# kije/HSLU_I.BA_RAYTRACING.F2501_raytracer

Hardware: AMD Instinct MI355X
Metric: Mray/s (primary+secondary, rays counted as the reference casts them), semesterbild@high_resolution (higher is better)
Workload: dtype f32; 1 GPU; semesterbild@high_resolution+anti_aliasing+soft_shadows (text.obj); width=1620, height=1350, rays_per_frame=34992000, rays_traced_per_frame=19683000, pixels_written=1768966, objects=14578, lights=50, parallelism=tiles48x48/1gpu, frames_in_flight=2, build_id=a7677b40f149b919-p0s0w0o6, queue_bytes=0, scene_budget_bytes=2147483648, phases=0

## Files before the change

hslu_i/ba_raytracing/f2501_raytracer_amd/csrc/rt_api.cpp:

```cpp
#include <hip/hip_runtime.h>

#include <algorithm>
#include <chrono>
#include <cmath>
#include <cstdio>
#include <cstdlib>
#include <cstring>
#include <string>
#include <vector>

#include "rt_cell_resolve.h"
#include "rt_host.h"

static void trace_point(hipStream_t stream, const char* what, uint32_t a = 0, uint32_t b = 0, uint32_t c = 0);
#define RC_TRY(expr) do { const int rc_ = (expr); if (rc_ != RT_OK) return rc_; } while (0)

extern "C" {

#ifndef RT_BUILD_ID
#define RT_BUILD_ID "unknown"
#endif
const char* rt_build_id(void) { return RT_BUILD_ID; }

int rt_selftest_exact_math(int device, const float* in, float* out_sqrt, float* out_rcp, uint32_t n) {
// ... 16 lines not shown
  if (e1 != hipSuccess || e2 != hipSuccess) return fail(RT_ERR_HIP, "selftest copy failed");
  return RT_OK;
}

int rt_device_count(void) {
  int n = 0;
  if (hipGetDeviceCount(&n) != hipSuccess) return 0;
  return n;
}

void rt_scene_destroy(rt_scene* s) {
  if (!s) return;
  (void)hipSetDevice(s->device);
  if (s->tables_ev) (void)hipEventDestroy(s->tables_ev);
  for (hipEvent_t e : s->frame_ev)
    if (e) (void)hipEventDestroy(e);
  for (auto& w : s->ws) {
    if (w.cnt_ev) (void)hipEventDestroy(w.cnt_ev);
    if (w.cnt_host) (void)hipHostFree(w.cnt_host);
    if (w.fork_ev) (void)hipEventDestroy(w.fork_ev);
    w.acc.release();
    for (auto& l : w.lane) {
      if (l.stream) (void)hipStreamSynchronize(l.stream), (void)hipStreamDestroy(l.stream);
      if (l.done_ev) (void)hipEventDestroy(l.done_ev);
      for (int k = 0; k < 2; k++) {
        if (l.shade_stream[k]) (void)hipStreamSynchronize(l.shade_stream[k]), (void)hipStreamDestroy(l.shade_stream[k]);
        if (l.shade_done[k]) (void)hipEventDestroy(l.shade_done[k]);
      }
      for (hipEvent_t e : l.level_ev) (void)hipEventDestroy(e);
      if (l.hit_ev) (void)hipEventDestroy(l.hit_ev);
      for (DevBuf* b : {&l.queues, &l.qcount, &l.trace_ws, &l.hard, &l.hitrec, &l.sets}) b->release();
    }
  }
  for (DevBuf* b : {&s->blob, &s->aa, &s->cloud, &s->counters, &s->suplist, &s->fb, &s->aux_rgb, &s->costmap, &s->aux_id, &s->aux_t, &s->flag_geo, &s->flags, &s->cell_lists, &s->resolve_work, &s->progress_fb, &s->rays_argb})
    b->release();
  rt_scene_release_update(s);
  delete s;
}

static int upload(DevBuf& b, const void* src, size_t bytes) {
  int rc = b.ensure(bytes);
  if (rc != RT_OK) return rc;
  if (bytes) {
    hipError_t e = hipMemcpy(b.p, src, bytes, hipMemcpyHostToDevice);
    if (e != hipSuccess) return fail(RT_ERR_HIP, "hipMemcpy H2D failed: %s", hipGetErrorString(e));
  }
  return RT_OK;
}

int rt_scene_create(const rt_scene_desc* d, int device, rt_scene** out) {
  if (!d || !out) return fail(RT_ERR_INVALID_ARG, "null argument");
  *out = nullptr;
  int rc = rt_check_scene_desc(d);
  if (rc != RT_OK) return rc;
  if ((rc = rt_open_device(device)) != RT_OK) return rc;

  rt_scene* s = new rt_scene();
  s->device = device;
  s->budget = d->device_budget_bytes ? d->device_budget_bytes : RT_SCENE_BUDGET_DEFAULT;
  RtPackedScene pk;
  rc = rt_pack_scene(d, s->budget, &pk);
  if (rc == RT_OK && pk.n_cells) {
    rc = upload(s->flag_geo, pk.flag_geo.data(), pk.flag_geo.size() * 4);
    if (rc == RT_OK) rc = s->flags.ensure((size_t)pk.n_cells * 2 + 64);
  }
  if (rc == RT_OK) rc = s->counters.ensure(RT_SLOTS * RT_COUNTER_REPLICAS * 16 * sizeof(unsigned long long));
  if (rc == RT_OK) rc = upload(s->blob, pk.blob.data(), pk.blob.size());
// ... 2 lines not shown
  if (rc == RT_OK) {
    rt_sah_packed(pk, s->sah_created, nullptr);
    s->sah_tri_cost = d->bvh.tri_cost > 0.f ? d->bvh.tri_cost : 2.0f;
  }
  if (rc != RT_OK) {
    rt_scene_destroy(s);
    return rc;
  }
  s->dev = pk.dev;
  s->dev.base = (const char*)s->blob.p;
  s->info = pk.info;
  s->n_cells = pk.n_cells;
  s->n_tri_cells = pk.n_tri_cells;
  s->bytes_bvh = pk.bytes_bvh;
  s->max_leaf = pk.max_leaf;
  memcpy(s->aabb_lo, pk.aabb_lo, sizeof(s->aabb_lo));
  memcpy(s->aabb_hi, pk.aabb_hi, sizeof(s->aabb_hi));
  *out = s;
  return RT_OK;
}

int rt_scene_bvh_info(const rt_scene* s, rt_bvh_info* out) {
  if (!s || !out) return fail(RT_ERR_INVALID_ARG, "null argument");
  *out = s->info;
  return RT_OK;
}

int rt_scene_memory_info(const rt_scene* s, rt_scene_info* out) {
  if (!s || !out) return fail(RT_ERR_INVALID_ARG, "null argument");
  memset(out, 0, sizeof(*out));
  out->bytes_bvh = s->bytes_bvh;
  out->bytes_geometry = s->blob.cap > s->bytes_bvh ? s->blob.cap - s->bytes_bvh : 0;
  out->bytes_flags = s->flags.cap + s->flag_geo.cap;
  out->bytes_cell_lists = s->cell_lists.cap + s->resolve_work.cap;
  out->bytes_tables = s->aa.cap + s->cloud.cap + s->counters.cap + s->suplist.cap + s->costmap.cap;
  for (const auto& w : s->ws) {
    out->bytes_workspace += w.bytes();
    for (const auto& l : w.lane) out->bytes_workspace += l.qcount.cap;
  }
  out->bytes_frames = s->fb.cap + s->aux_rgb.cap + s->aux_id.cap + s->aux_t.cap + s->progress_fb.cap + s->rays_argb.cap;
  out->bytes_total = out->bytes_geometry + out->bytes_bvh + out->bytes_flags + out->bytes_cell_lists + out->bytes_tables + out->bytes_workspace +
                     out->bytes_frames;
  out->budget_bytes = s->budget;
  out->n_receiver_cells = s->n_cells;
  out->cell_lists_built = s->cell_lists_built ? 1u : 0u;
  return RT_OK;
}

}

int rt_validate_params(const rt_params* p) {
  if (!p) return fail(RT_ERR_INVALID_ARG, "null params");
  if (p->abi_version != RT_ABI_VERSION)
    return fail(RT_ERR_INVALID_ARG, "rt_params.abi_version %u != %u", p->abi_version, RT_ABI_VERSION);
  if (p->width == 0 || p->height == 0) return fail(RT_ERR_INVALID_ARG, "empty frame");
  if ((uint64_t)p->width * p->height > 0x7FFFFFFFull) return fail(RT_ERR_INVALID_ARG, "frame too large");
  if (p->win_w && (p->win_x0 + (uint64_t)p->win_w > p->width || p->win_y0 + (uint64_t)p->win_h > p->height || !p->win_h))
    return fail(RT_ERR_INVALID_ARG, "window outside the frame");
  if ((p->flags & RT_FLAG_ANTI_ALIASING) && p->aa_rays > 0 && !p->aa_offsets)
    return fail(RT_ERR_INVALID_ARG, "aa_offsets missing");
  if (p->light_mult > 1 && (!p->cloud_sets || p->n_cloud_sets == 0))
    return fail(RT_ERR_INVALID_ARG, "cloud_sets missing");
  if (p->n_ranks > 1 && p->rank >= p->n_ranks) return fail(RT_ERR_INVALID_ARG, "rank out of range");
  if (p->n_ranks > 1 && p->tile_size != 0 && p->tile_size < 16) return fail(RT_ERR_UNSUPPORTED, "tile_size < 16");
  if (p->traversal > RT_TRAVERSAL_LINEAR) return fail(RT_ERR_INVALID_ARG, "unknown traversal mode");
  if (p->max_depth_reflection > RT_MAX_DEPTH || p->max_depth_refraction > RT_MAX_DEPTH)
    return fail(RT_ERR_UNSUPPORTED, "recursion depth > %u", RT_MAX_DEPTH);
// ... 87 lines not shown
    if (new_table) s->cloud_host.assign(p->cloud_sets, p->cloud_sets + n);
    s->cloud_ball_f[0] = p->fw, s->cloud_ball_f[1] = p->fh, s->cloud_ball_f[2] = p->fd;
    rt_scale_cloud(s->cloud_host.data(), n, s->cloud_ball_f, &s->cloud_scaled, s->cloud_ball);
    HIP_TRY(hipMemcpyAsync(s->cloud.p, s->cloud_scaled.data(), n / 3 * 16, hipMemcpyHostToDevice, up.stream));
  }
  P->cloud_sets = (const float4*)s->cloud.p;
  memcpy(P->cloud_centre, s->cloud_ball, 12);
  P->cloud_delta = s->cloud_ball[3];
  rt_beam_constants(p->eps_distance, P);
  const uint32_t cap = p->tuning.shadow_candidate_cap;
  P->cand_cap = cap == RT_CAND_CAP_NONE ? 0u : (cap ? cap : 64u);
  return RT_OK;
}

static int prepare_receiver_flags(rt_scene* s, const rt_params* p, TableUpload& up, RtDevParams* P) {
  hipStream_t stream = up.stream;
  P->recv_flags = nullptr;
  if (p->tuning.no_receiver_flags || P->cand_cap == 0u) s->notes |= RT_NOTE_RECV_FLAGS_OFF_TUNING;
  if (!s->n_cells || !(P->cloud_delta > 0.0f)) s->notes |= RT_NOTE_RECV_FLAGS_OFF_SCENE;
  if (s->dev.n_lights > 8u) s->notes |= RT_NOTE_RECV_FLAGS_OFF_LIGHTS;
  if (p->traversal != RT_TRAVERSAL_BVH) s->notes |= RT_NOTE_RECV_FLAGS_OFF_TRAVERSAL;
  if (p->flags & RT_FLAG_BACKFACE_CULLING) s->notes |= RT_NOTE_RECV_FLAGS_OFF_CULLING;
  if (!p->tuning.no_receiver_flags && P->cand_cap != 0u && s->n_cells && s->dev.n_lights <= 8u && p->traversal == RT_TRAVERSAL_BVH &&
      !(p->flags & RT_FLAG_BACKFACE_CULLING) && P->cloud_delta > 0.0f) {
    const float key[8] = {P->beam_delta, p->eps_distance, P->cloud_centre[0], P->cloud_centre[1], P->cloud_centre[2], 1.f, 0.f, 0.f};
    if (memcmp(key, s->flags_key, sizeof(key)) != 0) {
      RC_TRY(up.begin());
      RtDevParams B = *P;
      B.flag_out = (uint16_t*)s->flags.p;
      B.flag_geo = (const float4*)s->flag_geo.p;
      B.n_cells = s->n_cells;
      B.n_tri_cells = s->n_tri_cells;
      s->cell_lists_built = false;
      B.cell_list_out = nullptr;
      const size_t list_bytes = (size_t)s->n_cells * s->dev.n_lights * 16u;
      size_t free_b = 0, total_b = 0;
      const size_t flag_bytes = s->flags.cap + s->flag_geo.cap;
      if (s->dev.n_slots <= 65533u && flag_bytes + list_bytes <= s->budget && hipMemGetInfo(&free_b, &total_b) == hipSuccess &&
          list_bytes <= (free_b + s->cell_lists.cap) / 4 && s->cell_lists.ensure(list_bytes + 64) == RT_OK) {
        HIP_TRY(hipMemsetAsync(s->cell_lists.p, 0xFF, list_bytes, stream));
        B.cell_list_out = (uint16_t*)s->cell_lists.p;
        s->cell_lists_built = true;
      }
      if (!s->cell_lists_built) s->cell_lists.release();
      hipError_t e = (hipError_t)rt_launch_flags(s->dev, B, stream);
      if (e != hipSuccess) return fail(RT_ERR_HIP, "rt_flags_kernel launch failed: %s", hipGetErrorString(e));
      trace_point(stream, "rt_flags_kernel: cells, lights, lists", s->n_cells, s->dev.n_lights, s->cell_lists_built ? 1u : 0u);
      static const char* const prune_env = getenv("RT_CELL_PRUNE");
      static const bool prune_off = prune_env && *prune_env == '0';
      if (s->cell_lists_built && !prune_off) {
        RtCellPruneArgs a{};
        a.flag_geo = (const float*)s->flag_geo.p;
        a.lists = (uint16_t*)s->cell_lists.p;
        a.flags = (uint16_t*)s->flags.p;
        a.n_cells = s->n_cells, a.n_tri_cells = s->n_tri_cells;
        memcpy(a.cloud_centre, P->cloud_centre, 12);
        a.beam_delta = P->beam_delta, a.beam_eps_o = P->beam_eps_o;
        a.mode = RT_PRUNE_FULL;
        e = (hipError_t)rt_launch_cell_prune(s->dev, a, stream);
        if (e != hipSuccess) return fail(RT_ERR_HIP, "rt_cell_prune_kernel launch failed: %s", hipGetErrorString(e));
        trace_point(stream, "rt_cell_prune_kernel: cells, lights", s->n_cells, s->dev.n_lights, 0u);
        static const char* const resolve_env = getenv("RT_CELL_RESOLVE");
        static const bool resolve_off = resolve_env && *resolve_env == '0';
        RtCellResolveArgs r{};
        const size_t temp_bytes = resolve_off ? 0 : rt_cell_resolve_temp_bytes(s->n_cells, s->budget - flag_bytes - list_bytes, &r.chunk_cells);
        if (temp_bytes && s->resolve_work.ensure(temp_bytes) == RT_OK) {
          r.cell = a;
          r.eps_push = P->beam_eps_push, r.eps_ulp = P->beam_eps_ulp;
          r.work = (uint32_t*)s->resolve_work.p;
          e = (hipError_t)rt_launch_cell_resolve(s->dev, r, stream);
          if (e != hipSuccess) return fail(RT_ERR_HIP, "rt_cell_resolve_kernel launch failed: %s", hipGetErrorString(e));
          trace_point(stream, "rt_cell_resolve_kernel: cells, lights, cells per chunk", s->n_cells, s->dev.n_lights, r.chunk_cells);
        } else {
          s->resolve_work.release();
        }
      }
      if (!s->cell_lists_built) s->resolve_work.release();
      memcpy(s->flags_key, key, sizeof(key));
    }
    P->recv_flags = (const uint16_t*)s->flags.p;
    if (s->cell_lists_built && !p->tuning.no_cell_lists) P->cell_lists = (const uint4*)s->cell_lists.p;
  }
  if (!P->cell_lists) s->notes |= RT_NOTE_CELL_LISTS_OFF;
  return RT_OK;
}

static void copy_frame_shape(rt_scene* s, const rt_params* p, uint32_t* argb_dev, const rt_aux* aux_dev, RtDevParams* P) {
  P->max_depth_reflection = p->max_depth_reflection;
  P->max_depth_refraction = p->max_depth_refraction;
  s->sort_bits_wanted = p->tuning.sort_bits;
  s->lanes_wanted = p->tuning.sub_frames;
  s->phases_wanted = p->tuning.phases;
  s->levels_wanted = p->tuning.levels;
  if (p->win_w) {
    P->win_x0 = p->win_x0, P->win_y0 = p->win_y0, P->win_w = p->win_w, P->win_h = p->win_h;
  } else {
    P->win_x0 = P->win_y0 = 0;
    P->win_w = p->width;
    P->win_h = p->height;
  }
  P->tile_size = p->tile_size ? p->tile_size : 48u;
  P->n_ranks = p->n_ranks;
  P->rank = p->rank;
  P->traversal = p->traversal;
  P->argb = argb_dev;
  if (aux_dev) {
    P->aux_rgb = aux_dev->rgb;
    P->aux_hit_id = aux_dev->hit_id;
    P->aux_hit_t = aux_dev->hit_t;
  }
}

static int take_frame_slot(rt_scene* s, const rt_params* p, hipStream_t stream, RtDevParams* P) {
  int blk = -1, oldest = 0, same = -1;
// ... 767 lines not shown
```

hslu_i/ba_raytracing/f2501_raytracer_amd/csrc/rt_cell_resolve.cpp:

```cpp
#include <hip/hip_runtime_api.h>

#include "rt_cell_resolve.h"
#include "rt_scene_pack.h"

void rt_cell_resolve_packed(const RtPackedScene& pk, RtCellResolveArgs a) {
  if (pk.dev.n_lights == 0u || pk.dev.n_lights > 8u || pk.flag_geo.empty()) return;
  a.cell.flag_geo = pk.flag_geo.data();
  a.cell.n_cells = a.cell.n_cells < pk.n_cells ? a.cell.n_cells : pk.n_cells;
  a.cell.n_tri_cells = pk.n_tri_cells;
  const char* base = (const char*)pk.blob.data();
  const uint32_t nl = pk.dev.n_lights;
  for (uint32_t c = 0; c < a.cell.n_cells; c++)
    rt_cell_resolve_cell(pk.dev, base, a, c, a.cell.lists + (size_t)c * nl * RT_PRUNE_LIST_SLOTS, a.cell.flags + c, a.counts ? a.counts + (size_t)c * nl : nullptr);
}

size_t rt_cell_resolve_temp_bytes(uint32_t n_cells, size_t budget_left, uint32_t* chunk_cells) {
  *chunk_cells = 0u;
  const size_t cap = budget_left < ((size_t)64u << 20) ? budget_left : ((size_t)64u << 20);
  if (n_cells == 0u || cap < 4096u + 4u * 256u) return 0;
  size_t chunk = (cap - 4096u) / 4u;
  if (chunk > n_cells) chunk = n_cells;
  if (((size_t)n_cells + chunk - 1u) / chunk > 1024u) return 0;
  *chunk_cells = (uint32_t)chunk;
  return 4096u + 4u * chunk;
}
```

hslu_i/ba_raytracing/f2501_raytracer_amd/csrc/rt_cell_resolve.h:

```cpp
#pragma once

#include "rt_cell_prune.h"

#define RT_RESOLVE_NEAR_CENTRE 0x100u
#define RT_RESOLVE_NO_INFLATE 0x200u
#define RT_RESOLVE_NO_NEAR 0x400u

struct RtCellResolveArgs {
  RtCellPruneArgs cell;
  float eps_push, eps_ulp;
  uint32_t* work;
  uint32_t chunk_cells;
  uint8_t* counts;
};

struct RtResolveCell {
  float pm[3], pt[8][3];
  float rho, scale;
};

RT_HD static inline bool rt_resolve_cell_setup(const RtDevScene& sc, const char* base, const RtCellPruneArgs& a, uint32_t c, RtResolveCell& K) {
  float extra;
  if (!rt_prune_cell_hull(sc, base, a, c, K.pm, K.pt, &extra)) return false;
  float r = 0.0f, scale = rt_fadd(rt_prune_norm1(K.pm), extra);
  for (int k = 0; k < 8; k++) {
    float dk[3];
    rt_prune_sub(K.pt[k], K.pm, dk);
    r = fmaxf(r, rt_prune_norm(dk));
    scale = fmaxf(scale, rt_fadd(rt_prune_norm1(K.pt[k]), extra));
  }
  K.rho = rt_fadd(rt_fadd(rt_fmul(r, 1.0001f), rt_fmul(2e-6f, scale)), a.beam_eps_o);
  K.scale = scale;
  return true;
}
RT_HD static inline void rt_resolve_beam(const RtDevScene& sc, const char* base, const RtCellPruneArgs& a, const RtResolveCell& K, uint32_t l, RtPruneBeam& B) {
  const float* lights = (const float*)(base + sc.off_lights);
  B.p[0] = K.pm[0], B.p[1] = K.pm[1], B.p[2] = K.pm[2];
  B.rho = K.rho;
  for (int x = 0; x < 3; x++) B.c[x] = rt_fadd(lights[8u * l + x], a.cloud_centre[x]);
  rt_prune_sub(B.c, B.p, B.dseg);
  B.delta = rt_fadd(a.beam_delta, rt_fmul(2e-6f, rt_fadd(K.scale, rt_prune_norm1(B.c))));
  B.lenp = rt_fadd(rt_fadd(rt_prune_norm(B.dseg), B.delta), B.rho);
}

RT_HD static inline bool rt_resolve_near_rule(const RtPruneBeam& B, const RtResolveCell& K, const RtCellResolveArgs& a, const float* q) {
  const float v1[3] = {q[0], q[1], q[2]}, X[3] = {q[9], q[10], q[11]};
  float b[3];
// ... 66 lines not shown
      if (next <= node) return false;
      node = next;
    }
    if (k >= n) return true;
    const uint32_t slot = first + k;
    k++;
    if (slot >= sc.n_slots || slot >= RT_PRUNE_LIST_OVERFLOW) return false;
    const float* q = isect + 12u * (size_t)slot;
    if (rt_prune_rule(B, q, mode & 0xFFu)) continue;
    if (!(mode & RT_RESOLVE_NO_NEAR) && rt_resolve_near_rule(B, K, a, q)) continue;
    if (!keep(slot)) return true;
  }
}

RT_HD static inline bool rt_cell_resolve_wanted(const uint16_t* list, uint32_t n_lights) {
  bool any = false;
  for (uint32_t l = 0; l < n_lights && l < 8u; l++) any = any || list[(size_t)l * RT_PRUNE_LIST_SLOTS] == RT_PRUNE_LIST_OVERFLOW;
  return any;
}

RT_HD static inline void rt_cell_resolve_cell(const RtDevScene& sc, const char* base, const RtCellResolveArgs& a, uint32_t c, uint16_t* list, uint16_t* flag,
                                              uint8_t* counts) {
  if (!rt_cell_resolve_wanted(list, sc.n_lights)) return;
  RtResolveCell K;
  if (!rt_resolve_cell_setup(sc, base, a.cell, c, K)) return;
  uint32_t fl = *flag;
  bool fl_changed = false;
  for (uint32_t l = 0; l < sc.n_lights && l < 8u; l++) {
    uint16_t* w = list + (size_t)l * RT_PRUNE_LIST_SLOTS;
    if (w[0] != RT_PRUNE_LIST_OVERFLOW) continue;
    RtPruneBeam B;
    rt_resolve_beam(sc, base, a.cell, K, l, B);
    uint32_t n = 0;
    uint16_t out[RT_PRUNE_LIST_SLOTS];
    const bool count_all = counts != nullptr;
    const bool ok = rt_resolve_walk(sc, base, a, K, B, [&](uint32_t slot) {
      if (n < RT_PRUNE_LIST_SLOTS) out[n] = (uint16_t)slot;
      n++;
      return n <= RT_PRUNE_LIST_SLOTS || count_all;
    });
    if (!ok) continue;
    if (counts) counts[l] = (uint8_t)(n < 255u ? n : 255u);
    if (n > RT_PRUNE_LIST_SLOTS) continue;
    for (uint32_t k = n; k < RT_PRUNE_LIST_SLOTS; k++) out[k] = (uint16_t)RT_PRUNE_LIST_END;
    memcpy(__builtin_assume_aligned(w, 16), out, 16);
    if (n == 0u) fl |= 1u << l, fl_changed = true;
  }
  if (fl_changed) *flag = (uint16_t)fl;
}

struct RtPackedScene;
void rt_cell_resolve_packed(const RtPackedScene& pk, RtCellResolveArgs a);
size_t rt_cell_resolve_temp_bytes(uint32_t n_cells, size_t budget_left, uint32_t* chunk_cells);
int rt_launch_cell_resolve(const RtDevScene& sc, const RtCellResolveArgs& a, void* stream);
```

hslu_i/ba_raytracing/f2501_raytracer_amd/csrc/rt_cell_resolve.hip:

```cpp
#include <hip/hip_runtime.h>

#include "rt_cell_resolve.h"

#define RT_CELL_RESOLVE_WG 256u
#define RT_CELL_RESOLVE_COUNTERS 1024u

__global__ __launch_bounds__(RT_CELL_RESOLVE_WG) void rt_cell_resolve_find_kernel(const uint16_t* lists, uint32_t n_lights, uint32_t cell0, uint32_t cell1,
                                                                                  uint32_t* counter, uint32_t* work) {
  const uint32_t c = cell0 + blockIdx.x * RT_CELL_RESOLVE_WG + threadIdx.x;
  const bool has = c < cell1 && rt_cell_resolve_wanted(lists + (size_t)c * n_lights * RT_PRUNE_LIST_SLOTS, n_lights);
  const unsigned long long m = __ballot(has);
  if (!m) return;
  const uint32_t lane = threadIdx.x & 63u, leader = (uint32_t)__ffsll((long long)m) - 1u;
  uint32_t at = 0u;
  if (lane == leader) at = atomicAdd(counter, (uint32_t)__popcll(m));
  at = (uint32_t)__shfl((int)at, (int)leader);
  if (has) work[at + (uint32_t)__popcll(m & ((1ull << lane) - 1ull))] = c;
}

__global__ __launch_bounds__(RT_CELL_RESOLVE_WG) void rt_cell_resolve_kernel(RtDevScene sc, RtCellResolveArgs a, const uint32_t* counter, const uint32_t* work) {
  const uint32_t i = blockIdx.x * RT_CELL_RESOLVE_WG + threadIdx.x;
  if (i >= *counter || i >= a.chunk_cells) return;
  const uint32_t c = work[i];
  if (c >= a.cell.n_cells) return;
  rt_cell_resolve_cell(sc, sc.base, a, c, a.cell.lists + (size_t)c * sc.n_lights * RT_PRUNE_LIST_SLOTS, a.cell.flags + c,
                       a.counts ? a.counts + (size_t)c * sc.n_lights : nullptr);
}

int rt_launch_cell_resolve(const RtDevScene& sc, const RtCellResolveArgs& a, void* stream) {
  const uint32_t n = a.cell.n_cells, chunk = a.chunk_cells;
  if (n == 0u || sc.n_lights == 0u || sc.n_lights > 8u || sc.n_thr == 0u) return 0;
  if (!a.work || chunk == 0u || ((size_t)n + chunk - 1u) / chunk > RT_CELL_RESOLVE_COUNTERS) return (int)hipErrorInvalidValue;
  hipStream_t st = (hipStream_t)stream;
  hipError_t e = hipMemsetAsync(a.work, 0, RT_CELL_RESOLVE_COUNTERS * 4u, st);
  if (e != hipSuccess) return (int)e;
  uint32_t* list = a.work + RT_CELL_RESOLVE_COUNTERS;
  uint32_t k = 0;
  for (uint32_t c0 = 0; c0 < n; k++) {
    const uint32_t c1 = n - c0 > chunk ? c0 + chunk : n;
    const dim3 grid((c1 - c0 + RT_CELL_RESOLVE_WG - 1u) / RT_CELL_RESOLVE_WG);
    hipLaunchKernelGGL(rt_cell_resolve_find_kernel, grid, dim3(RT_CELL_RESOLVE_WG), 0, st, a.cell.lists, sc.n_lights, c0, c1, a.work + k, list);
    hipLaunchKernelGGL(rt_cell_resolve_kernel, grid, dim3(RT_CELL_RESOLVE_WG), 0, st, sc, a, a.work + k, list);
    if ((e = hipGetLastError()) != hipSuccess) return (int)e;
    c0 = c1;
  }
  return 0;
}
```

hslu_i/ba_raytracing/f2501_raytracer_amd/csrc/rt_host.h:

```cpp
#pragma once

#include <hip/hip_runtime.h>

#include <string>
#include <vector>

#include "rt_closest.h"
#include "rt_multihit.h"
#include "rt_ray_key.h"
#include "rt_scene_pack.h"

#define fail rt_fail

#define HIP_TRY(expr)                                                                          \
  do {                                                                                         \
    hipError_t e_ = (expr);                                                                    \
    if (e_ != hipSuccess)                                                                      \
      return fail(e_ == hipErrorOutOfMemory ? RT_ERR_OOM : RT_ERR_HIP, "%s failed: %s", #expr, \
                  hipGetErrorString(e_));                                                      \
  } while (0)

#define RT_SLOTS 4
#define RT_LANES 2
#define RT_MAX_DEPTH 64u
// ... 219 lines not shown
    }
  } ws[RT_SLOTS];
  std::vector<uint32_t> sup_host;
  uint32_t sup_key[8] = {0, 0, 0, 0, 0, 0, 0, 0};
  DevBuf costmap;
  std::vector<uint32_t> cost_host;
  uint32_t cost_key[13] = {0, 0, 0, 0, 0, 0, 0, 0, 0, 0, 0, 0, 0};
  bool cost_valid = false, cost_wanted = false;
  uint32_t q_cap = 0, hard_cap = 0, batch_items = 0;
  StreamKey stream_key{};
  uint32_t key_gen = 0;
  uint32_t sticky_notes = 0;
  bool stream_verified = false;
  uint32_t est[RT_LANES][RT_CNT_STRIDE] = {{0}};
  bool est_valid = false;
  uint32_t sort_bits_wanted = 0;
  uint32_t lanes_wanted = 0;
  uint32_t phases_wanted = 0;
  uint32_t levels_wanted = 0;
  uint32_t calm_frames = 1u << 30;
  uint32_t tables_version = 0;
  float aabb_lo[3] = {0.f, 0.f, 0.f}, aabb_hi[3] = {1.f, 1.f, 1.f};
  std::vector<float> aa_host, cloud_host, cloud_scaled;
  std::vector<uint32_t> aa_table;
  uint32_t aa_unique = 0;
  bool aa_dedup = true;
  hipEvent_t tables_ev = nullptr;
  hipStream_t tables_stream = nullptr, last_stream = nullptr;
  bool tables_pending = false, rendered = false;
  float cloud_ball[4] = {0.f, 0.f, 0.f, -1.f};
  DevBuf flag_geo, flags;
  DevBuf cell_lists;
  DevBuf resolve_work;
  bool cell_lists_built = false;
  uint32_t n_cells = 0, n_tri_cells = 0;
  float flags_key[8] = {-1.f, 0.f, 0.f, 0.f, 0.f, 0.f, 0.f, 0.f};
  float cloud_ball_f[3] = {0.f, 0.f, 0.f};
  hipEvent_t frame_ev[RT_SLOTS] = {};
  bool frame_pending[RT_SLOTS] = {};
  uint32_t frame_seq[RT_SLOTS] = {};
  hipStream_t frame_stream[RT_SLOTS] = {};
  uint32_t frame_no = 0;
  int cur_block = 0, last_block = 0;
  int cur_ws = 0;
  int ws_last_block[RT_SLOTS] = {0, 1, 2, 3};
  uint32_t notes = 0;
  size_t queue_bytes = 0;
  RtRefitPlan plan;
  DevBuf plan_dev, upd_dev;
  size_t plan_off[5] = {0, 0, 0, 0, 0};
  void* upd_stage = nullptr;
  size_t upd_stage_cap = 0;
  float* upd_back = nullptr;
  uint64_t sah_created[2] = {0, 0};
  float sah_tri_cost = 2.0f;
  DevBuf sah_dev;
  uint32_t max_leaf = 4;
};


int rt_scene_upload_plan(rt_scene* s, const RtPackedScene& pk);
void rt_scene_release_update(rt_scene* s);

int rt_scene_wait_frames(rt_scene* s);

struct RtRebuildIn {
// ... 30 lines not shown
```

hslu_i/ba_raytracing/f2501_raytracer_amd/csrc/rt_internal.h:

```cpp
#pragma once

#include <stdint.h>

#include <vector>

#include "../../../../include/rt_hip.h"


struct RtNode {
  float lo0[3];
  uint32_t c0;
  float hi0[3];
  uint32_t n0;
  float lo1[3];
  uint32_t c1;
  float hi1[3];
  uint32_t n1;
};
static_assert(sizeof(RtNode) == 64, "node must be 64 bytes");

struct RtThrNode {
  float lo[3];
  uint32_t skip;
  float hi[3];
// ... 26 lines not shown
  uint32_t off_tri_shade;
  uint32_t off_tri_id;
  uint32_t off_materials;
  uint32_t off_lights;
  uint32_t off_nodes;
  uint32_t off_nodes_oct;
  uint32_t off_nodes_thr;
  uint32_t off_recv;
  uint32_t off_srecv;
  uint32_t n_thr;
  uint32_t n_spheres, n_triangles, n_lights, n_nodes;
  uint32_t n_slots;
};

struct RtDevParams {
  uint32_t width, height;
  float focus[3];
  float fw, fh, fd, eps_distance, air_ior, ambient;
  uint32_t flags;
  uint32_t aa_rays;
  uint32_t aa_unique;
  uint32_t weighted;
  const float* aa_offsets;
  const uint32_t* aa_mult;
  const uint32_t* aa_src;
  uint32_t light_mult, cloud_seed, n_cloud_sets;
  float beam_delta, beam_delta_e5, beam_eps_push, beam_eps_ulp, beam_eps_o, beam_eps_198;
  const float4* cloud_sets;
  float cloud_centre[3];
  float cloud_delta;
  uint32_t cand_cap;
  const uint16_t* recv_flags;
  const uint4* cell_lists;
  uint16_t* cell_list_out;
  uint16_t* flag_out;
  const float4* flag_geo;
  uint32_t n_cells;
  uint32_t n_tri_cells;
  uint32_t max_depth_reflection, max_depth_refraction;
  uint32_t win_x0, win_y0, win_w, win_h;
  uint32_t tile_size, n_ranks, rank;
  uint32_t traversal;
  const uint32_t* stage_slot;
  uint32_t stage_tiles_x;
  uint32_t* argb;
  float* aux_rgb;
  int32_t* aux_hit_id;
  float* aux_hit_t;
  unsigned long long* counters;
  float4* q_out;
  uint32_t* q_out_count;
  uint32_t* q_overflow;
  uint32_t q_capacity;
  float4* q_in;
  const uint32_t* q_in_count;
  long long* acc;
  float4* hard_q;
  uint32_t* hard_count;
  uint32_t* hard_stat;
  uint32_t hard_capacity;
  uint32_t* sort_hist;
  uint32_t* sort_offs;
  uint32_t* sort_tile;
  uint32_t* sort_hits;
  uint32_t* sh_idx;
  uint2* sort_slot;
  uint32_t sort_bits;
// ... 130 lines not shown
```

hslu_i/ba_raytracing/f2501_raytracer_amd/csrc/rt_kernels.hip:

```cpp
#include <hip/hip_runtime.h>

#include <stdlib.h>

#include <type_traits>

#include "rt_internal.h"

#define RT_EPS 1.1920929e-7f

#define RT_OPAQUE(v) asm volatile("" : "+v"(v))
#define RT_OPAQUE_S(v) asm volatile("" : "+s"(v))
typedef const __attribute__((address_space(4))) char* rt_kernarg_ptr;
__device__ __forceinline__ rt_kernarg_ptr kernarg_fresh() {
  rt_kernarg_ptr p = (rt_kernarg_ptr)__builtin_amdgcn_kernarg_segment_ptr();
  asm volatile("" : "+s"(p));
  return p;
}
#define RT_KERNARG_OFF_P ((sizeof(RtDevScene) + alignof(RtDevParams) - 1) / alignof(RtDevParams) * alignof(RtDevParams))
static_assert(RT_KERNARG_OFF_P == 88, "RtDevParams follows RtDevScene at kernarg offset 88");
__device__ __forceinline__ const RtDevScene& kernarg_scene() { return *(const RtDevScene*)(const char*)kernarg_fresh(); }
__device__ __forceinline__ const RtDevParams& kernarg_params() {
  return *(const RtDevParams*)((const char*)kernarg_fresh() + RT_KERNARG_OFF_P);
}
#define wave_ballot(pred) __builtin_amdgcn_ballot_w64((bool)(pred))
// ... 462 lines not shown
__device__ __forceinline__ lanemask shadow_accumulate_lane(Shadow& S, const Mat& m, V3 n, V3 d, lanemask h) {
  if (CULL) h &= wave_ballot(m.transmissive || dot(d, n) < 0.75f);
  S.occ |= h & wave_ballot(!m.transmissive);
  const float io = m.transmissive ? m.opacity * (1.0f - fresnel_reflectance_air_red(m, n, -d)) : 0.0f;
  const bool on = lane_of(h);
  const uint32_t di = (uint32_t)__float2uint_rn(clampf(1.0f - io, 0.0f, 1.0f) * RT_SH_SCALE);
  const uint32_t nd = min(S.dec + di, RT_SH_ONE);
  S.dec = on ? nd : S.dec;
  const V3 ab = absorption(m);
  S.fr = on ? S.fr + (uint32_t)__float2uint_rn(ab.x * RT_FILT_SCALE) : S.fr;
  S.fg = on ? S.fg + (uint32_t)__float2uint_rn(ab.y * RT_FILT_SCALE) : S.fg;
  S.fb = on ? S.fb + (uint32_t)__float2uint_rn(ab.z * RT_FILT_SCALE) : S.fb;
  return h;
}

struct WaveCtx {
  uint32_t n_nodes, n_tris, s_nodes, s_tris, s_passes, n_exact, s_exact;
  uint32_t o_exec, o_miss;
#if RT_PROFILE
  unsigned long long t_mark;
  unsigned long long prof[7];
#endif
};

enum { CFG_TABLES_RUNTIME = -1, CFG_TABLES_FLAGS = 1, CFG_TABLES_LISTS = 2 };
struct CfgGeneric {
  static constexpr uint32_t N = 0u;
  static constexpr bool BVH = false;
  static constexpr int TABLES = CFG_TABLES_RUNTIME;
  static constexpr bool POW2_SETS = false;
  static constexpr bool FEW_SPHERES = false;
  static constexpr bool FAR_ORIGINS = false;
  static constexpr bool OCC_MEMO = false;
};
template <uint32_t N_, int TABLES_>
struct CfgSoft {
  static constexpr uint32_t N = N_;
  static constexpr bool BVH = true;
  static constexpr int TABLES = TABLES_;
  static constexpr bool POW2_SETS = true;
  static constexpr bool FEW_SPHERES = true;
  static constexpr bool FAR_ORIGINS = false;
  static constexpr bool OCC_MEMO = TABLES_ == CFG_TABLES_LISTS;
};
struct CfgRays : CfgGeneric {
  static constexpr bool FAR_ORIGINS = true;
};

template <bool CULL, class C = CfgGeneric>
__device__ __forceinline__ Hit nearest_hit(const RtDevScene& sc, const RtDevParams& P, WaveCtx& W,
                                           bool alive, V3 o, V3 d) {
  Hit best;
  best.t = INFINITY;
  best.id = -1;
  const lanemask grp = wave_ballot(alive);
  uint32_t pre = 0xFFFFFFFFu;
  if (sc.n_spheres > 2u && grp) {
    const uint32_t ns = C::FEW_SPHERES ? sc.n_spheres : (sc.n_spheres < 32u ? sc.n_spheres : 32u);
    const int fl = __ffsll((long long)grp) - 1;
    auto first = [&](float v) { return __uint_as_float((uint32_t)__builtin_amdgcn_readlane((int)__float_as_uint(v), fl)); };
    const V3 o0 = mk(first(o.x), first(o.y), first(o.z)), d0 = mk(first(d.x), first(d.y), first(d.z));
    const V3 eo = o - o0, ed = d - d0;
    float so = alive ? fabsf(eo.x) + fabsf(eo.y) + fabsf(eo.z) : 0.0f, sd = alive ? fabsf(ed.x) + fabsf(ed.y) + fabsf(ed.z) : 0.0f;
#pragma unroll
    for (int k = 32; k >= 1; k >>= 1) {
      so = fmaxf(so, __shfl_xor(so, k, 64));
      sd = fmaxf(sd, __shfl_xor(sd, k, 64));
    }
    const uint32_t lane = threadIdx.x & 63u, si = lane < ns ? lane : ns - 1u;
    const float4 sp = vload<float4>(sc, sc.off_spheres + si * 16u);
    const float rad = vload<float>(sc, sc.off_sphere_rad + si * 4u);
    const V3 w = mk(sp.x, sp.y, sp.z) - o0;
    const float tc = fmaxf(dot(w, d0), 0.0f);
    const V3 q = w - d0 * tc;
    const float reach = rad + so + (mag(w) + so + rad) * sd * 1.0001f + 1e-6f;
    pre = (uint32_t)(wave_ballot(dot(q, q) <= reach * reach * 1.0002f) & ((1ull << ns) - 1ull));
// ... 124 lines not shown
        next = (uint32_t)__builtin_amdgcn_readlane((int)stk, (int)sp);
      }
      node = next;
    }
  };
  if (octant_uniform)
    walk(std::true_type{});
  else
    walk(std::false_type{});
  return best;
}

#define RT_MAX_CANDIDATES 64u
#define RT_CAND_OVERFLOW 0xFFFFFFFFu

struct CandList {
  uint32_t reg;
  uint32_t count;
  uint32_t spheres;
  unsigned long long umbra;
#if RT_PROFILE == 5
  uint32_t own;
#endif
};

struct FatBeam {
  float r;
  V3 pt[8];
  uint16_t* list;
};
#define RT_CELL_LIST_SLOTS 8u
#define RT_CELL_LIST_END 0xFFFFu
#define RT_CELL_LIST_OVERFLOW 0xFFFEu
enum { COLLECT_OWN = 0, COLLECT_FLAGS = 1 };

template <bool CULL, int MODE = COLLECT_OWN, class C = CfgGeneric>
__device__ __forceinline__ CandList collect_light_candidates(const RtDevScene& sc, WaveCtx& W, bool alive, V3 p, V3 c,
                                                              const RtDevParams& P, V3 p_first, float p_spread, uint32_t cand_cap,
                                                              const FatBeam* fb = nullptr, bool walk_tris = true,
                                                              bool have_pre = false, uint32_t pre_reg = 0, uint32_t pre_count = 0) {
  RT_OPAQUE_S(cand_cap);
  const float delta = MODE == COLLECT_FLAGS ? P.beam_delta + fb->r : P.beam_delta;
  const float delta_e5 = MODE == COLLECT_FLAGS ? P.beam_delta_e5 + fb->r : P.beam_delta_e5;
  CandList L;
  L.reg = 0;
  L.count = 0;
  L.spheres = 0xFFFFFFFFu;
  L.umbra = 0ull;
#if RT_PROFILE == 5
  L.own = 0;
#endif
  const uint32_t lane_id = threadIdx.x & 63u;
  V3 dseg = c - p;
  float len = fmaxf(mag(dseg), 1e-20f);
  V3 inv = mk(clampf(__builtin_amdgcn_rcpf(dseg.x), -1e30f, 1e30f), clampf(__builtin_amdgcn_rcpf(dseg.y), -1e30f, 1e30f),
              clampf(__builtin_amdgcn_rcpf(dseg.z), -1e30f, 1e30f));
  V3 noi = mk(-(p.x * inv.x), -(p.y * inv.y), -(p.z * inv.z));
  V3 dl = mk(delta * fabsf(inv.x), delta * fabsf(inv.y), delta * fabsf(inv.z));
  float send = 1.0f + delta_e5 * __builtin_amdgcn_rcpf(len) + 1e-5f;
  float sbeg = -(delta_e5 * __builtin_amdgcn_rcpf(len) + 1e-5f);
  const V3 cn = noi - dl, cf = noi + dl;
  auto box = [&](const float* lo, const float* hi, float& smin) {
    smin = fmaxf(fmaxf(fminf(__builtin_fmaf(lo[0], inv.x, cn.x), __builtin_fmaf(hi[0], inv.x, cn.x)),
                       fminf(__builtin_fmaf(lo[1], inv.y, cn.y), __builtin_fmaf(hi[1], inv.y, cn.y))),
                 fminf(__builtin_fmaf(lo[2], inv.z, cn.z), __builtin_fmaf(hi[2], inv.z, cn.z)));
    float smax = fminf(fminf(fmaxf(__builtin_fmaf(lo[0], inv.x, cf.x), __builtin_fmaf(hi[0], inv.x, cf.x)),
// ... 888 lines not shown
      const float scale = fabsf(dc.x) + fabsf(dc.y) + fabsf(dc.z) + fabsf(sf.p.x) + fabsf(sf.p.y) + fabsf(sf.p.z) + 1.0f;
      use = hit && (dot(sf.n, dc) + n1 * __builtin_fmaf(4e-6f, scale, dl) > 0.0f);
    }
    lanemask use_m = wave_ballot(use);
    if (!use_m) {
      continue;
    }
    CandList cand = cand_unknown();
#if RT_PROFILE == 4
    uint32_t prof_walked = 0, prof_listed = 0, prof_pre = 0;
#endif
    if ((RT_SKIP & 4) && N > 1) {
      cand.count = 0;
      cand.spheres = 0;
    } else if (N > 1 && (C::BVH || P.cloud_delta > 0.0f) && (C::BVH || P.traversal == RT_TRAVERSAL_BVH) && (C::BVH || sc.n_triangles)) {
      V3 centre = mk(L0.x + P.cloud_centre[0], L0.y + P.cloud_centre[1], L0.z + P.cloud_centre[2]);
      const unsigned long long t_c = PROF_T();
      bool walk_tris = true, test_spheres = true;
      if (!CULL && (C::TABLES != CFG_TABLES_RUNTIME || P.recv_flags)) {
        uint32_t tix = threadIdx.x;
        RT_OPAQUE(tix);
        const uint32_t rf = __float_as_uint(stash[10u * 256u + tix]) >> l;
        walk_tris = (use_m & ~wave_ballot(rf & 1u)) != 0ull;
        test_spheres = walk_tris || (use_m & ~wave_ballot((rf >> 8) & 1u)) != 0ull;
      }
      uint32_t pre_reg = 0, pre_count = 0;
      bool have_pre = false;
      if (!CULL && (C::TABLES == CFG_TABLES_LISTS || (C::TABLES == CFG_TABLES_RUNTIME && P.cell_lists)) && walk_tris) {
        uint32_t tix = threadIdx.x;
        RT_OPAQUE(tix);
        const uint32_t cidx = __float_as_uint(stash[RT_STASH_CELL * 256u + tix]);
        uint4 lst = make_uint4(0xFFFFFFFFu, 0xFFFFFFFFu, 0xFFFFFFFFu, 0xFFFFFFFFu);
        if (use && cidx != RT_NO_CELL) lst = P.cell_lists[(size_t)cidx * sc.n_lights + l];
        const lanemask unusable = use_m & (wave_ballot(cidx == RT_NO_CELL) | wave_ballot((lst.x & 0xFFFFu) == RT_CELL_LIST_OVERFLOW));
        if (!unusable) {
          have_pre = true;
          const uint32_t lane_id = threadIdx.x & 63u;
          for (lanemask todo = use_m & ~wave_ballot((lst.x & 0xFFFFu) == RT_CELL_LIST_END); todo;) {
            const int fl = __ffsll((long long)todo) - 1;
            const uint32_t c = (uint32_t)__builtin_amdgcn_readlane((int)cidx, fl);
            auto add_slot = [&](uint32_t slot) {
              if (slot >= RT_CELL_LIST_OVERFLOW) return;
              const lanemask filled = pre_count >= 64u ? ~0ull : ((1ull << pre_count) - 1ull);
              if (wave_ballot(pre_reg == slot) & filled) return;
              lane_put(pre_reg, pre_count, slot, lane_id);
              pre_count++;
            };
            auto add_pair = [&](uint32_t v) {
              const uint32_t w = (uint32_t)__builtin_amdgcn_readlane((int)v, fl);
              add_slot(w & 0xFFFFu);
              add_slot(w >> 16);
            };
            add_pair(lst.x), add_pair(lst.y), add_pair(lst.z), add_pair(lst.w);
            todo &= ~wave_ballot(cidx == c);
          }
          if (pre_count > 64u) have_pre = false;
        }
      }
#if RT_PROFILE == 4
      prof_walked = (walk_tris && !have_pre) ? 1u : 0u, prof_listed = have_pre ? 1u : 0u, prof_pre = have_pre ? pre_count : 0u;
#endif
      if (test_spheres) {
        cand = collect_light_candidates<CULL, COLLECT_OWN, C>(sc, W, use, sf.p, centre, P, p_first, p_spread, P.cand_cap, nullptr, walk_tris,
                                                              have_pre, pre_reg, pre_count);
      } else {
        cand.count = 0;
        cand.spheres = 0;
      }
#if RT_PROFILE
      RT_OPAQUE(cand.reg);
#endif
      PROF_ADD(W, 1, t_c);
#if RT_SKIP
      if (RT_SKIP & 1) cand.spheres = 0;
      if (RT_SKIP & 2) cand.count = 0;
      if ((RT_SKIP & 8) && cand.count == RT_CAND_OVERFLOW) cand.count = 0, cand.spheres = 0;
#endif
#if RT_PROFILE == 2
      {
        const uint32_t nsph = (uint32_t)__popc(cand.spheres & ((1u << (sc.n_spheres < 32u ? sc.n_spheres : 31u)) - 1u));
        const bool ov = cand.count == RT_CAND_OVERFLOW;
        W.prof[0] += (!ov && cand.count == 0 && nsph == 0) ? 1 : 0;
        W.prof[1] += (!ov && cand.count == 0 && nsph > 0) ? 1 : 0;
        W.prof[2] += (!ov && cand.count >= 1 && cand.count <= 4) ? 1 : 0;
        W.prof[3] += (!ov && cand.count >= 5 && cand.count <= 16) ? 1 : 0;
        W.prof[4] += (!ov && cand.count > 16) ? 1 : 0;
        W.prof[5] += ov ? 1 : 0;
        W.prof[6] += nsph;
      }
#endif
    }
    if (cand.umbra) {
      use_m &= ~cand.umbra;
// ... 1134 lines not shown
```

Measured before the change: 8676 Mray/s.

## Add wide overflow records for per-cell light candidate lists

```diff
diff --git a/hslu_i/ba_raytracing/f2501_raytracer_amd/csrc/rt_api.cpp b/hslu_i/ba_raytracing/f2501_raytracer_amd/csrc/rt_api.cpp
--- a/hslu_i/ba_raytracing/f2501_raytracer_amd/csrc/rt_api.cpp
+++ b/hslu_i/ba_raytracing/f2501_raytracer_amd/csrc/rt_api.cpp
@@ -72,7 +72,7 @@
       for (DevBuf* b : {&l.queues, &l.qcount, &l.trace_ws, &l.hard, &l.hitrec, &l.sets}) b->release();
     }
   }
-  for (DevBuf* b : {&s->blob, &s->aa, &s->cloud, &s->counters, &s->suplist, &s->fb, &s->aux_rgb, &s->costmap, &s->aux_id, &s->aux_t, &s->flag_geo, &s->flags, &s->cell_lists, &s->resolve_work, &s->progress_fb, &s->rays_argb})
+  for (DevBuf* b : {&s->blob, &s->aa, &s->cloud, &s->counters, &s->suplist, &s->fb, &s->aux_rgb, &s->costmap, &s->aux_id, &s->aux_t, &s->flag_geo, &s->flags, &s->cell_lists, &s->resolve_work, &s->cell_wide, &s->progress_fb, &s->rays_argb})
     b->release();
   rt_scene_release_update(s);
   delete s;
@@ -141,7 +141,7 @@
   out->bytes_bvh = s->bytes_bvh;
   out->bytes_geometry = s->blob.cap > s->bytes_bvh ? s->blob.cap - s->bytes_bvh : 0;
   out->bytes_flags = s->flags.cap + s->flag_geo.cap;
-  out->bytes_cell_lists = s->cell_lists.cap + s->resolve_work.cap;
+  out->bytes_cell_lists = s->cell_lists.cap + s->resolve_work.cap + s->cell_wide.cap;
   out->bytes_tables = s->aa.cap + s->cloud.cap + s->counters.cap + s->suplist.cap + s->costmap.cap;
   for (const auto& w : s->ws) {
     out->bytes_workspace += w.bytes();
@@ -295,6 +295,7 @@
       B.n_cells = s->n_cells;
       B.n_tri_cells = s->n_tri_cells;
       s->cell_lists_built = false;
+      s->cell_wide_built = false;
       B.cell_list_out = nullptr;
       const size_t list_bytes = (size_t)s->n_cells * s->dev.n_lights * 16u;
       size_t free_b = 0, total_b = 0;
@@ -331,6 +332,18 @@
           r.cell = a;
           r.eps_push = P->beam_eps_push, r.eps_ulp = P->beam_eps_ulp;
           r.work = (uint32_t*)s->resolve_work.p;
+          static const char* const wide_env = getenv("RT_CELL_WIDE");
+          static const bool wide_off = wide_env && *wide_env == '0';
+          const size_t used = flag_bytes + list_bytes + temp_bytes;
+          const size_t wide_bytes = wide_off || used >= s->budget ? 0 : rt_cell_wide_pool_bytes(s->n_cells, s->dev.n_lights, s->budget - used, &r.wide_cap);
+          if (wide_bytes && hipMemGetInfo(&free_b, &total_b) == hipSuccess && wide_bytes <= (free_b + s->cell_wide.cap) / 4 &&
+              s->cell_wide.ensure(wide_bytes) == RT_OK) {
+            r.wide = (uint16_t*)s->cell_wide.p;
+            r.wide_count = (uint32_t*)((char*)s->cell_wide.p + (size_t)r.wide_cap * 2u * RT_CELL_WIDE_SLOTS);
+            s->cell_wide_built = true;
+          } else {
+            r.wide_cap = 0u;
+          }
           e = (hipError_t)rt_launch_cell_resolve(s->dev, r, stream);
           if (e != hipSuccess) return fail(RT_ERR_HIP, "rt_cell_resolve_kernel launch failed: %s", hipGetErrorString(e));
           trace_point(stream, "rt_cell_resolve_kernel: cells, lights, cells per chunk", s->n_cells, s->dev.n_lights, r.chunk_cells);
@@ -339,10 +352,12 @@
         }
       }
       if (!s->cell_lists_built) s->resolve_work.release();
+      if (!s->cell_wide_built) s->cell_wide.release();
       memcpy(s->flags_key, key, sizeof(key));
     }
     P->recv_flags = (const uint16_t*)s->flags.p;
     if (s->cell_lists_built && !p->tuning.no_cell_lists) P->cell_lists = (const uint4*)s->cell_lists.p;
+    if (P->cell_lists && s->cell_wide_built) P->cell_wide = (const uint32_t*)s->cell_wide.p;
   }
   if (!P->cell_lists) s->notes |= RT_NOTE_CELL_LISTS_OFF;
   return RT_OK;
diff --git a/hslu_i/ba_raytracing/f2501_raytracer_amd/csrc/rt_cell_resolve.cpp b/hslu_i/ba_raytracing/f2501_raytracer_amd/csrc/rt_cell_resolve.cpp
--- a/hslu_i/ba_raytracing/f2501_raytracer_amd/csrc/rt_cell_resolve.cpp
+++ b/hslu_i/ba_raytracing/f2501_raytracer_amd/csrc/rt_cell_resolve.cpp
@@ -24,3 +24,15 @@
   *chunk_cells = (uint32_t)chunk;
   return 4096u + 4u * chunk;
 }
+
+size_t rt_cell_wide_pool_bytes(uint32_t n_cells, uint32_t n_lights, size_t budget_left, uint32_t* wide_cap) {
+  *wide_cap = 0u;
+  const size_t rec = 2u * RT_CELL_WIDE_SLOTS;
+  if (n_cells == 0u || n_lights == 0u || budget_left < 2u * rec) return 0;
+  size_t cap = (budget_left - rec) / rec;
+  const size_t lists = (size_t)n_cells * n_lights;
+  if (cap > (lists + 7u) / 8u) cap = (lists + 7u) / 8u;
+  if (cap > RT_CELL_WIDE_MAX_RECORDS) cap = RT_CELL_WIDE_MAX_RECORDS;
+  *wide_cap = (uint32_t)cap;
+  return cap * rec + rec;
+}
diff --git a/hslu_i/ba_raytracing/f2501_raytracer_amd/csrc/rt_cell_resolve.h b/hslu_i/ba_raytracing/f2501_raytracer_amd/csrc/rt_cell_resolve.h
--- a/hslu_i/ba_raytracing/f2501_raytracer_amd/csrc/rt_cell_resolve.h
+++ b/hslu_i/ba_raytracing/f2501_raytracer_amd/csrc/rt_cell_resolve.h
@@ -5,6 +5,10 @@
 #define RT_RESOLVE_NEAR_CENTRE 0x100u
 #define RT_RESOLVE_NO_INFLATE 0x200u
 #define RT_RESOLVE_NO_NEAR 0x400u
+
+#define RT_CELL_WIDE_SLOTS 32u
+#define RT_CELL_WIDE_MARK 0xFFFDu
+#define RT_CELL_WIDE_MAX_RECORDS (1u << 30)
 
 struct RtCellResolveArgs {
   RtCellPruneArgs cell;
@@ -12,7 +16,24 @@
   uint32_t* work;
   uint32_t chunk_cells;
   uint8_t* counts;
+  uint16_t* wide;
+  uint32_t wide_cap;
+  uint32_t* wide_count;
 };
+
+RT_HD static inline uint32_t rt_cell_wide_index(const uint16_t* w) {
+  if (w[0] != RT_PRUNE_LIST_OVERFLOW || w[1] != RT_CELL_WIDE_MARK) return ~0u;
+  return (uint32_t)(w[2] & 0x7FFFu) | ((uint32_t)(w[3] & 0x7FFFu) << 15);
+}
+RT_HD static inline uint32_t rt_cell_wide_take(const RtCellResolveArgs& a) {
+  if (!a.wide || !a.wide_count || a.wide_cap == 0u) return ~0u;
+#if defined(__HIP_DEVICE_COMPILE__)
+  const uint32_t at = __hip_atomic_fetch_add(a.wide_count, 1u, __ATOMIC_RELAXED, __HIP_MEMORY_SCOPE_AGENT);
+#else
+  const uint32_t at = (*a.wide_count)++;
+#endif
+  return at < a.wide_cap && at < RT_CELL_WIDE_MAX_RECORDS ? at : ~0u;
+}
 
 struct RtResolveCell {
   float pm[3], pt[8][3];
@@ -145,16 +166,27 @@
     RtPruneBeam B;
     rt_resolve_beam(sc, base, a.cell, K, l, B);
     uint32_t n = 0;
-    uint16_t out[RT_PRUNE_LIST_SLOTS];
+    uint16_t out[RT_CELL_WIDE_SLOTS];
     const bool count_all = counts != nullptr;
+    const uint32_t room = a.wide ? RT_CELL_WIDE_SLOTS : RT_PRUNE_LIST_SLOTS;
     const bool ok = rt_resolve_walk(sc, base, a, K, B, [&](uint32_t slot) {
-      if (n < RT_PRUNE_LIST_SLOTS) out[n] = (uint16_t)slot;
+      if (n < room) out[n] = (uint16_t)slot;
       n++;
-      return n <= RT_PRUNE_LIST_SLOTS || count_all;
+      return n <= room || count_all;
     });
     if (!ok) continue;
     if (counts) counts[l] = (uint8_t)(n < 255u ? n : 255u);
-    if (n > RT_PRUNE_LIST_SLOTS) continue;
+    if (n > room) continue;
+    if (n > RT_PRUNE_LIST_SLOTS) {
+      const uint32_t at = rt_cell_wide_take(a);
+      if (at == ~0u) continue;
+      for (uint32_t k = n; k < RT_CELL_WIDE_SLOTS; k++) out[k] = (uint16_t)RT_PRUNE_LIST_END;
+      memcpy(__builtin_assume_aligned(a.wide + (size_t)at * RT_CELL_WIDE_SLOTS, 64), out, 2u * RT_CELL_WIDE_SLOTS);
+      const uint16_t mark[RT_PRUNE_LIST_SLOTS] = {(uint16_t)RT_PRUNE_LIST_OVERFLOW, (uint16_t)RT_CELL_WIDE_MARK, (uint16_t)(at & 0x7FFFu), (uint16_t)((at >> 15) & 0x7FFFu),
+                                                  (uint16_t)RT_PRUNE_LIST_END, (uint16_t)RT_PRUNE_LIST_END, (uint16_t)RT_PRUNE_LIST_END, (uint16_t)RT_PRUNE_LIST_END};
+      memcpy(__builtin_assume_aligned(w, 16), mark, 16);
+      continue;
+    }
     for (uint32_t k = n; k < RT_PRUNE_LIST_SLOTS; k++) out[k] = (uint16_t)RT_PRUNE_LIST_END;
     memcpy(__builtin_assume_aligned(w, 16), out, 16);
     if (n == 0u) fl |= 1u << l, fl_changed = true;
@@ -165,4 +197,5 @@
 struct RtPackedScene;
 void rt_cell_resolve_packed(const RtPackedScene& pk, RtCellResolveArgs a);
 size_t rt_cell_resolve_temp_bytes(uint32_t n_cells, size_t budget_left, uint32_t* chunk_cells);
+size_t rt_cell_wide_pool_bytes(uint32_t n_cells, uint32_t n_lights, size_t budget_left, uint32_t* wide_cap);
 int rt_launch_cell_resolve(const RtDevScene& sc, const RtCellResolveArgs& a, void* stream);
diff --git a/hslu_i/ba_raytracing/f2501_raytracer_amd/csrc/rt_cell_resolve.hip b/hslu_i/ba_raytracing/f2501_raytracer_amd/csrc/rt_cell_resolve.hip
--- a/hslu_i/ba_raytracing/f2501_raytracer_amd/csrc/rt_cell_resolve.hip
+++ b/hslu_i/ba_raytracing/f2501_raytracer_amd/csrc/rt_cell_resolve.hip
@@ -34,6 +34,7 @@
   hipStream_t st = (hipStream_t)stream;
   hipError_t e = hipMemsetAsync(a.work, 0, RT_CELL_RESOLVE_COUNTERS * 4u, st);
   if (e != hipSuccess) return (int)e;
+  if (a.wide && a.wide_count && (e = hipMemsetAsync(a.wide_count, 0, 4u, st)) != hipSuccess) return (int)e;
   uint32_t* list = a.work + RT_CELL_RESOLVE_COUNTERS;
   uint32_t k = 0;
   for (uint32_t c0 = 0; c0 < n; k++) {
diff --git a/hslu_i/ba_raytracing/f2501_raytracer_amd/csrc/rt_host.h b/hslu_i/ba_raytracing/f2501_raytracer_amd/csrc/rt_host.h
--- a/hslu_i/ba_raytracing/f2501_raytracer_amd/csrc/rt_host.h
+++ b/hslu_i/ba_raytracing/f2501_raytracer_amd/csrc/rt_host.h
@@ -275,6 +275,8 @@
   DevBuf flag_geo, flags;
   DevBuf cell_lists;
   DevBuf resolve_work;
+  DevBuf cell_wide;
+  bool cell_wide_built = false;
   bool cell_lists_built = false;
   uint32_t n_cells = 0, n_tri_cells = 0;
   float flags_key[8] = {-1.f, 0.f, 0.f, 0.f, 0.f, 0.f, 0.f, 0.f};
diff --git a/hslu_i/ba_raytracing/f2501_raytracer_amd/csrc/rt_internal.h b/hslu_i/ba_raytracing/f2501_raytracer_amd/csrc/rt_internal.h
--- a/hslu_i/ba_raytracing/f2501_raytracer_amd/csrc/rt_internal.h
+++ b/hslu_i/ba_raytracing/f2501_raytracer_amd/csrc/rt_internal.h
@@ -82,7 +82,10 @@
   uint32_t cand_cap;
   const uint16_t* recv_flags;
   const uint4* cell_lists;
-  uint16_t* cell_list_out;
+  union {
+    uint16_t* cell_list_out;
+    const uint32_t* cell_wide;
+  };
   uint16_t* flag_out;
   const float4* flag_geo;
   uint32_t n_cells;
diff --git a/hslu_i/ba_raytracing/f2501_raytracer_amd/csrc/rt_kernels.hip b/hslu_i/ba_raytracing/f2501_raytracer_amd/csrc/rt_kernels.hip
--- a/hslu_i/ba_raytracing/f2501_raytracer_amd/csrc/rt_kernels.hip
+++ b/hslu_i/ba_raytracing/f2501_raytracer_amd/csrc/rt_kernels.hip
@@ -518,6 +518,7 @@
   static constexpr bool FEW_SPHERES = false;
   static constexpr bool FAR_ORIGINS = false;
   static constexpr bool OCC_MEMO = false;
+  static constexpr bool WIDE = false;
 };
 template <uint32_t N_, int TABLES_>
 struct CfgSoft {
@@ -528,6 +529,7 @@
   static constexpr bool FEW_SPHERES = true;
   static constexpr bool FAR_ORIGINS = false;
   static constexpr bool OCC_MEMO = TABLES_ == CFG_TABLES_LISTS;
+  static constexpr bool WIDE = TABLES_ == CFG_TABLES_LISTS;
 };
 struct CfgRays : CfgGeneric {
   static constexpr bool FAR_ORIGINS = true;
@@ -718,6 +720,8 @@
 #define RT_CELL_LIST_SLOTS 8u
 #define RT_CELL_LIST_END 0xFFFFu
 #define RT_CELL_LIST_OVERFLOW 0xFFFEu
+#define RT_CELL_WIDE_HEAD 0xFFFDFFFEu
+#define RT_CELL_WIDE_DWORDS 16u
 enum { COLLECT_OWN = 0, COLLECT_FLAGS = 1 };
 
 template <bool CULL, int MODE = COLLECT_OWN, class C = CfgGeneric>
@@ -1672,11 +1676,12 @@
         const uint32_t cidx = __float_as_uint(stash[RT_STASH_CELL * 256u + tix]);
         uint4 lst = make_uint4(0xFFFFFFFFu, 0xFFFFFFFFu, 0xFFFFFFFFu, 0xFFFFFFFFu);
         if (use && cidx != RT_NO_CELL) lst = P.cell_lists[(size_t)cidx * sc.n_lights + l];
-        const lanemask unusable = use_m & (wave_ballot(cidx == RT_NO_CELL) | wave_ballot((lst.x & 0xFFFFu) == RT_CELL_LIST_OVERFLOW));
+        const lanemask wide_m = C::WIDE ? use_m & wave_ballot(lst.x == RT_CELL_WIDE_HEAD) : 0ull;
+        const lanemask unusable = use_m & (wave_ballot(cidx == RT_NO_CELL) | wave_ballot((lst.x & 0xFFFFu) == RT_CELL_LIST_OVERFLOW)) & ~wide_m;
         if (!unusable) {
           have_pre = true;
           const uint32_t lane_id = threadIdx.x & 63u;
-          for (lanemask todo = use_m & ~wave_ballot((lst.x & 0xFFFFu) == RT_CELL_LIST_END); todo;) {
+          for (lanemask todo = use_m & ~wave_ballot((lst.x & 0xFFFFu) == RT_CELL_LIST_END) & ~wide_m; todo;) {
             const int fl = __ffsll((long long)todo) - 1;
             const uint32_t c = (uint32_t)__builtin_amdgcn_readlane((int)cidx, fl);
             auto add_slot = [&](uint32_t slot) {
@@ -1694,11 +1699,67 @@
             add_pair(lst.x), add_pair(lst.y), add_pair(lst.z), add_pair(lst.w);
             todo &= ~wave_ballot(cidx == c);
           }
+          if constexpr (C::WIDE) {
+            if (__builtin_expect(wide_m != 0ull, 0))
+            for (lanemask todo = wide_m; todo;) {
+              const int fl = __ffsll((long long)todo) - 1;
+              const uint32_t c = (uint32_t)__builtin_amdgcn_readlane((int)cidx, fl);
+              const uint32_t iw = (uint32_t)__builtin_amdgcn_readlane((int)lst.y, fl);
+              const uint4* rec = (const uint4*)(P.cell_wide + (size_t)((iw & 0x7FFFu) | ((iw >> 1) & 0x3FFF8000u)) * RT_CELL_WIDE_DWORDS);
+              auto add_slot = [&](uint32_t slot) {
+                if (slot >= RT_CELL_LIST_OVERFLOW) return;
+                const lanemask filled = pre_count >= 64u ? ~0ull : ((1ull << pre_count) - 1ull);
+                if (wave_ballot(pre_reg == slot) & filled) return;
+                lane_put(pre_reg, pre_count, slot, lane_id);
+                pre_count++;
+              };
+              auto put_slot = [&](uint32_t slot) {
+                if (slot >= RT_CELL_LIST_OVERFLOW) return;
+                lane_put(pre_reg, pre_count, slot, lane_id);
+                pre_count++;
+              };
+              const bool fresh = pre_count == 0u;
+              for (uint32_t k = 0; k < RT_CELL_WIDE_DWORDS / 4u; k++) {
+                const uint4 q = uload(rec + k);
+                if (fresh) {
+                  put_slot(q.x & 0xFFFFu), put_slot(q.x >> 16), put_slot(q.y & 0xFFFFu), put_slot(q.y >> 16);
+                  put_slot(q.z & 0xFFFFu), put_slot(q.z >> 16), put_slot(q.w & 0xFFFFu), put_slot(q.w >> 16);
+                } else {
+                  add_slot(q.x & 0xFFFFu), add_slot(q.x >> 16), add_slot(q.y & 0xFFFFu), add_slot(q.y >> 16);
+                  add_slot(q.z & 0xFFFFu), add_slot(q.z >> 16), add_slot(q.w & 0xFFFFu), add_slot(q.w >> 16);
+                }
+                if ((q.w >> 16) == RT_CELL_LIST_END) break;
+              }
+              todo &= ~wave_ballot(cidx == c);
+            }
+          }
           if (pre_count > 64u) have_pre = false;
         }
       }
 #if RT_PROFILE == 4
       prof_walked = (walk_tris && !have_pre) ? 1u : 0u, prof_listed = have_pre ? 1u : 0u, prof_pre = have_pre ? pre_count : 0u;
+#endif
+#if RT_PROFILE == 6
+      if (!CULL && (C::TABLES == CFG_TABLES_LISTS || (C::TABLES == CFG_TABLES_RUNTIME && P.cell_lists)) && walk_tris) {
+        uint32_t tix = threadIdx.x;
+        RT_OPAQUE(tix);
+        const uint32_t cidx = __float_as_uint(stash[RT_STASH_CELL * 256u + tix]);
+        uint4 lst = make_uint4(0xFFFFFFFFu, 0xFFFFFFFFu, 0xFFFFFFFFu, 0xFFFFFFFFu);
+        if (use && cidx != RT_NO_CELL) lst = P.cell_lists[(size_t)cidx * sc.n_lights + l];
+        const bool is_wide = C::WIDE && lst.x == RT_CELL_WIDE_HEAD;
+        const lanemask nocell_m = use_m & wave_ballot(cidx == RT_NO_CELL);
+        const lanemask plain_m = use_m & wave_ballot((lst.x & 0xFFFFu) == RT_CELL_LIST_OVERFLOW && !is_wide);
+        const lanemask wide_m = use_m & wave_ballot(is_wide);
+        bool longer = false;
+        if (use && is_wide) longer = (P.cell_wide[(size_t)((lst.y & 0x7FFFu) | ((lst.y >> 1) & 0x3FFF8000u)) * RT_CELL_WIDE_DWORDS + 8u] & 0xFFFFu) != RT_CELL_LIST_END;
+        W.prof[0] += have_pre ? 0u : 1u;
+        W.prof[1] += (!have_pre && nocell_m) ? 1u : 0u;
+        W.prof[2] += (!have_pre && !nocell_m && plain_m) ? 1u : 0u;
+        W.prof[3] += (!have_pre && !nocell_m && !plain_m) ? 1u : 0u;
+        W.prof[4] += (have_pre && wide_m) ? 1u : 0u;
+        W.prof[5] += (have_pre && wide_m && !wave_ballot(longer)) ? 1u : 0u;
+        W.prof[6] += have_pre ? 1u : 0u;
+      }
 #endif
       if (test_spheres) {
         cand = collect_light_candidates<CULL, COLLECT_OWN, C>(sc, W, use, sf.p, centre, P, p_first, p_spread, P.cand_cap, nullptr, walk_tris,
```

After: 8790 Mray/s (median of 6 runs). 1.01x the previous value.
